# flatironinstitute/bayes-kit

Measured on NVIDIA B200. Metric: hmc_chain_steps_per_s, higher is better.
Workload: dtype f32

## Files before the change

bayes-kit_b200/csrc/dense_tc.cu:

```cuda
#include <cuda.h>
#include <cuda_bf16.h>
#include <stdio.h>
#include <stdlib.h>

#include <mutex>

#include "dense_tc.h"
#include "sep_common.cuh"

namespace bk {

namespace tc {

constexpr int BM = 128;
constexpr int BN = 256;
constexpr int BK = 64;
constexpr int UK = 16;
constexpr int CWID = 16;
constexpr int EDEPTH_MAX = 4;
constexpr int ECHUNK_BYTES = 2 * CWID * 32 * 4;
template <int MODE, bool PAIR = false> struct Cfg {
    static constexpr int KS = MODE == TC_MODE_STEP ? 32 : 64;
#ifndef BK_STEP_STAGES
#define BK_STEP_STAGES 8
// ... 505 lines not shown
                                const float qn = qj + fmaf(em2, gj, qj - pj);
                                __stcs(qw + j * BM, qn);
                                const __nv_bfloat16 hi = __float2bfloat16_rn(qn);
                                hw[j * BK] = hi;
                                lw[j * BK] = __float2bfloat16_rn(qn - __bfloat162float(hi));
                            }
                        }
                    } else if (!no_mem) {
#pragma unroll
                        for (int j = 0; j < CWID; ++j) {
                            float pj, qj;
                            asm volatile("ld.shared.f32 %0, [%1];" : "=f"(pj) : "r"(src + j * 128));
                            asm volatile("ld.shared.f32 %0, [%1];" : "=f"(qj) : "r"(src + CWID * 128 + j * 128));
                            if (d_ok && cbase + ch * CWID + j < a.C) {
                                const float gj = cv - __uint_as_float(v[j]);
                                const float qn = qj + fmaf(em2, gj, qj - pj);
                                __stcs(qw + j * BM, qn);
                                const __nv_bfloat16 hi = __float2bfloat16_rn(qn);
                                hw[j * BK] = hi;
                                if (lw) lw[j * BK] = __float2bfloat16_rn(qn - __bfloat162float(hi));
                            }
                        }
                    }
                    qw += CWID * BM;
                    hw += CWID * BK;
                    if (lw) lw += CWID * BK;
                    src += ECHUNK_BYTES;
                    if (++slot == EDEPTH) { slot = 0; src -= EDEPTH * ECHUNK_BYTES; }
                    __syncwarp();
                };
                static_assert(NC % 2 == 0, "two register sets ping-pong");
                uint32_t va[CWID], vb[CWID];
                const bool no_tmem = (a.debug & 16) != 0;
                if (!no_tmem) tmem_ld16_async(t0, va);
#pragma unroll 1
                for (int ch = 0; ch < NC; ch += 2) {
                    issue();
                    cp_async_wait<EDEPTH - 1>();
                    __syncwarp();
                    tmem_wait_ld16(va);
                    if (!no_tmem) tmem_ld16_async(t0 + (ch + 1) * CWID, vb);
                    process(va, ch);
                    issue();
                    cp_async_wait<EDEPTH - 1>();
                    __syncwarp();
                    tmem_wait_ld16(vb);
                    if (ch + 2 < NC && !no_tmem) tmem_ld16_async(t0 + (ch + 2) * CWID, va);
                    process(vb, ch + 1);
                }
                if (!d_ok && !no_mem) {
                    hw -= NC * CWID * BK;
                    if (lw) lw -= NC * CWID * BK;
                    for (int j = 0; j < NCH * 32; ++j)
                        if (cbase + j < a.C) {
                            hw[(int64_t)j * BK] = __float2bfloat16_rn(0.f);
                            if (lw) lw[(int64_t)j * BK] = __float2bfloat16_rn(0.f);
                        }
                }
                tc_fence_before();
                if constexpr (PAIR) {
                    if (step < n_steps - 1) fence_proxy_async_global();
                    __syncwarp();
                    if (lane == 0) {
                        mbar_arrive_cluster(mapa_rank(tempty(acc), 0));
                        if (step < n_steps - 1) mbar_arrive(twritten(sig_k));
                    }
                    ++sig_k;
                } else {
                    mbar_arrive(tempty(acc));
                }
                if (++acc == 2) { acc = 0; acc_phase ^= 1u; }
            }
            cp_async_wait<0>();
        }
    }
    tc_fence_before();
    __syncthreads();
    if constexpr (PAIR) cluster_sync_all();
    if (warp == 1) {
        tc_fence_after();
        if constexpr (PAIR)
            asm volatile("tcgen05.dealloc.cta_group::2.sync.aligned.b32 %0, %1;" ::"r"(tmem_base), "r"(TMEM_COLS)
                         : "memory");
        else
            asm volatile("tcgen05.dealloc.cta_group::1.sync.aligned.b32 %0, %1;" ::"r"(tmem_base), "r"(TMEM_COLS)
                         : "memory");
    }
}

__global__ void k_split_matrix(const float* __restrict__ P, int D, int Dp, __nv_bfloat16* __restrict__ hi,
                               __nv_bfloat16* __restrict__ lo) {
    int64_t i = (int64_t)blockIdx.x * blockDim.x + threadIdx.x;
    if (i >= (int64_t)Dp * Dp) return;
    int r = (int)(i / Dp), c = (int)(i % Dp);
    float v = (r < D && c < D) ? P[(int64_t)r * D + c] : 0.0f;
    __nv_bfloat16 h = __float2bfloat16_rn(v);
    const int64_t o = box_index(r, c, Dp / BK, BM);
    hi[o] = h;
    lo[o] = __float2bfloat16_rn(v - __bfloat162float(h));
}

__global__ void k_pmu(const float* __restrict__ P, const float* __restrict__ mu, int D, float* __restrict__ out) {
    int r = (int)(((int64_t)blockIdx.x * blockDim.x + threadIdx.x) >> 5), lane = threadIdx.x & 31;
    if (r >= D) return;
    double s = 0;
    for (int k = lane; k < D; k += 32) s += (double)P[(int64_t)r * D + k] * (double)mu[k];
    s = warp_sum(s);
    if (lane == 0) out[r] = (float)s;
}

__global__ void k_split_rows(const float* __restrict__ x, int64_t C, int D, int Dp,
                             __nv_bfloat16* __restrict__ hi, __nv_bfloat16* __restrict__ lo) {
    int64_t i = (int64_t)blockIdx.x * blockDim.x + threadIdx.x;
    if (i >= C * Dp) return;
    int64_t c = i / Dp;
    int d = (int)(i % Dp);
    float v = d < D ? x[c * D + d] : 0.f;
    __nv_bfloat16 h = __float2bfloat16_rn(v);
    const int64_t o = box_index(c, d, Dp / BK, BN);
    hi[o] = h;
    if (lo) lo[o] = __float2bfloat16_rn(v - __bfloat162float(h));
}

struct HmcTcArgs {
    float *theta, *lp, *grad;
    float *q, *qm, *gq, *h0;
    __nv_bfloat16 *q_hi, *q_lo;
    const float *metric, *mu;
    int64_t C;
    int D, Dp, L, m_tiles;
    float eps, half_eps, inv_eps;
    bk_rng rng;
    float *draws, *logp;
    int32_t* accept;
    int out_lp;
    const uint32_t* err;
    const float *qs, *gs;
    int old_blocked;
    __nv_bfloat16 *nq_hi, *nq_lo;
};

template <bool VEC>
__device__ __forceinline__ void ld4(const float* p, int e, int D, float (&v)[4]) {
    if (VEC) {
        const float4 t = *reinterpret_cast<const float4*>(p + e);
        v[0] = t.x; v[1] = t.y; v[2] = t.z; v[3] = t.w;
    } else {
#pragma unroll
        for (int i = 0; i < 4; ++i) v[i] = (e + i < D) ? p[e + i] : 0.f;
    }
}
template <bool VEC>
__device__ __forceinline__ void st4(float* p, int e, int D, const float (&v)[4]) {
    if (VEC) {
        *reinterpret_cast<float4*>(p + e) = make_float4(v[0], v[1], v[2], v[3]);
    } else {
#pragma unroll
        for (int i = 0; i < 4; ++i)
            if (e + i < D) p[e + i] = v[i];
    }
}
template <bool VEC>
__device__ __forceinline__ void st4_bf16(__nv_bfloat16* p, int e, int D, const __nv_bfloat16 (&v)[4]) {
    if (VEC) {
        uint2 u;
        u.x = (uint32_t)__bfloat16_as_ushort(v[0]) | ((uint32_t)__bfloat16_as_ushort(v[1]) << 16);
        u.y = (uint32_t)__bfloat16_as_ushort(v[2]) | ((uint32_t)__bfloat16_as_ushort(v[3]) << 16);
        *reinterpret_cast<uint2*>(p + e) = u;
    } else {
#pragma unroll
        for (int i = 0; i < 4; ++i)
            if (e + i < D) p[e + i] = v[i];
    }
}

template <bool VEC>
__global__ void __launch_bounds__(256) k_hmc_begin_tc(HmcTcArgs p, int64_t t, int write_lo) {
    const int64_t c = ((int64_t)blockIdx.x * blockDim.x + threadIdx.x) >> 5;
    const int lane = threadIdx.x & 31;
    if (c >= p.C) return;
    const int D = p.D;
    const int64_t off = c * (int64_t)D;
    float kin = 0.f;
#pragma unroll 2
    for (int b = lane; 4 * b < D; b += 32) {
        const int e = 4 * b;
        float z[4], g[4], th[4], m[4] = {1.f, 1.f, 1.f, 1.f};
        ld4<VEC>(p.grad + off, e, D, g);
        ld4<VEC>(p.theta + off, e, D, th);
        if (p.metric) ld4<VEC>(p.metric, e, D, m);
        if (p.rng.mode == BK_RNG_INJECTED)
            ld4<VEC>(reinterpret_cast<const float*>(p.rng.normals) + (t * p.C + c) * (int64_t)D, e, D, z);
        else
            philox_normal4<float>(p.rng.seed, (uint32_t)b, (uint32_t)(p.rng.chain_offset + (uint64_t)c),
                                  (uint32_t)(p.rng.draw_offset + (uint64_t)t), z);
        float r[4], q[4];
        __nv_bfloat16 hi[4], lo[4];
#pragma unroll
        for (int i = 0; i < 4; ++i) {
            if (!VEC && e + i >= D) z[i] = 0.f;
            const float mg = m[i] * g[i];
            kin = fmaf(z[i], m[i] * z[i], kin);
            r[i] = z[i] - p.half_eps * mg;
            r[i] = r[i] + p.eps * mg;
            q[i] = th[i] + p.eps * r[i];
            hi[i] = __float2bfloat16_rn(q[i]);
            lo[i] = __float2bfloat16_rn(q[i] - __bfloat162float(hi[i]));
        }
        const int64_t bo = blk_index(c, e, p.m_tiles);
        st4<true>(p.qm + bo, 0, 4, th);
        st4<true>(p.q + bo, 0, 4, q);
        const int64_t xo = box_index(c, e, p.Dp / BK, BN);
        st4_bf16<true>(p.q_hi + xo, 0, 4, hi);
        if (write_lo) st4_bf16<true>(p.q_lo + xo, 0, 4, lo);
    }
    for (int b = (D + 3) / 4 + lane; 4 * b < p.Dp; b += 32) {
        const __nv_bfloat16 zero4[4] = {__float2bfloat16_rn(0.f), __float2bfloat16_rn(0.f), __float2bfloat16_rn(0.f),
                                        __float2bfloat16_rn(0.f)};
        const int64_t xo = box_index(c, 4 * b, p.Dp / BK, BN);
        st4_bf16<true>(p.q_hi + xo, 0, 4, zero4);
        if (write_lo) st4_bf16<true>(p.q_lo + xo, 0, 4, zero4);
    }
    kin = warp_sum(kin);
    if (lane == 0) p.h0[c] = p.lp[c] - 0.5f * kin;
}

template <bool VEC>
__global__ void __launch_bounds__(256) k_hmc_end_tc(HmcTcArgs p, int64_t t) {
    const int64_t c = ((int64_t)blockIdx.x * blockDim.x + threadIdx.x) >> 5;
    const int lane = threadIdx.x & 31;
    if (c >= p.C) return;
    const int D = p.D;
    const int64_t off = c * (int64_t)D;
    float kin = 0.f, dot = 0.f;
#pragma unroll 2
    for (int b = lane; 4 * b < D; b += 32) {
        const int e = 4 * b;
        float g[4], qm[4], q[4], m[4] = {1.f, 1.f, 1.f, 1.f}, mu[4] = {0.f, 0.f, 0.f, 0.f};
        const int64_t bo = blk_index(c, e, p.m_tiles);
        ld4<true>(p.gq + bo, 0, 4, g);
        ld4<true>(p.qm + bo, 0, 4, qm);
        ld4<true>(p.q + bo, 0, 4, q);
        if (p.metric) ld4<VEC>(p.metric, e, D, m);
        if (p.mu) ld4<VEC>(p.mu, e, D, mu);
#pragma unroll
        for (int i = 0; i < 4; ++i) {
            if (e + i >= D) break;
            const float rf = fmaf(q[i] - qm[i], p.inv_eps, p.half_eps * (m[i] * g[i]));
            kin = fmaf(rf, m[i] * rf, kin);
            dot = fmaf(q[i] - mu[i], g[i], dot);
        }
    }
    kin = warp_sum(kin);
    dot = warp_sum(dot);
    const bool lost = p.err && *p.err != 0u;
    const float lpq = lost ? __int_as_float(0x7fc00000) : 0.5f * dot;
    const float h1 = lpq - 0.5f * kin, h0 = lost ? lpq : p.h0[c];
    float u;
    if (p.rng.mode == BK_RNG_INJECTED)
        u = reinterpret_cast<const float*>(p.rng.uniforms)[(t * p.C + c) * p.rng.n_uniform];
    else
        u = philox_accept_uniform<float>(p.rng.seed, (uint32_t)(p.rng.chain_offset + (uint64_t)c),
                                         (uint32_t)(p.rng.draw_offset + (uint64_t)t), D);
    const bool acc = log_u(u) < h1 - h0;
    float* dr = p.draws ? p.draws + (t * p.C + c) * (int64_t)D : nullptr;
#pragma unroll 2
    for (int b = lane; 4 * b < D; b += 32) {
        const int e = 4 * b;
        float v[4];
        if (acc) {
            float g[4];
            const int64_t bo = blk_index(c, e, p.m_tiles);
            ld4<true>(p.q + bo, 0, 4, v);
            ld4<true>(p.gq + bo, 0, 4, g);
            st4<VEC>(p.theta + off, e, D, v);
            st4<VEC>(p.grad + off, e, D, g);
        } else if (p.old_blocked) {
            float g[4];
            const int64_t bo = blk_index(c, e, p.m_tiles);
            ld4<true>(p.qs + bo, 0, 4, v);
            ld4<true>(p.gs + bo, 0, 4, g);
            st4<VEC>(p.theta + off, e, D, v);
            st4<VEC>(p.grad + off, e, D, g);
        } else if (dr) {
            ld4<VEC>(p.theta + off, e, D, v);
        }
        if (dr) st4<VEC>(dr, e, D, v);
    }
    if (lane == 0) {
        const float lp_old = p.lp[c];
        if (acc) p.lp[c] = lpq;
        if (p.logp) p.logp[t * p.C + c] = p.out_lp ? (acc ? lpq : lp_old) : (acc ? h1 : h0);
        if (p.accept) p.accept[t * p.C + c] = acc ? 1 : 0;
    }
}

template <bool VEC>
__global__ void __launch_bounds__(256, 4) k_hmc_turn_tc(HmcTcArgs p, int64_t t, int write_lo) {
    const int64_t c = ((int64_t)blockIdx.x * blockDim.x + threadIdx.x) >> 5;
    const int lane = threadIdx.x & 31;
    if (c >= p.C) return;
    const int D = p.D;
    const int64_t off = c * (int64_t)D;
    float kin = 0.f, dot = 0.f;
#pragma unroll 2
    for (int b = lane; 4 * b < D; b += 32) {
        const int e = 4 * b;
        float g[4], qm[4], q[4], m[4] = {1.f, 1.f, 1.f, 1.f}, mu[4] = {0.f, 0.f, 0.f, 0.f};
        const int64_t bo = blk_index(c, e, p.m_tiles);
        ld4<true>(p.gq + bo, 0, 4, g);
        ld4<true>(p.qm + bo, 0, 4, qm);
        ld4<true>(p.q + bo, 0, 4, q);
        if (p.metric) ld4<VEC>(p.metric, e, D, m);
        if (p.mu) ld4<VEC>(p.mu, e, D, mu);
#pragma unroll
        for (int i = 0; i < 4; ++i) {
            if (e + i >= D) break;
            const float rf = fmaf(q[i] - qm[i], p.inv_eps, p.half_eps * (m[i] * g[i]));
            kin = fmaf(rf, m[i] * rf, kin);
            dot = fmaf(q[i] - mu[i], g[i], dot);
        }
    }
    kin = warp_sum(kin);
    dot = warp_sum(dot);
    const bool lost = p.err && *p.err != 0u;
    const float lpq = lost ? __int_as_float(0x7fc00000) : 0.5f * dot;
    const float h1 = lpq - 0.5f * kin, h0 = lost ? lpq : p.h0[c];
    float u;
    if (p.rng.mode == BK_RNG_INJECTED)
        u = reinterpret_cast<const float*>(p.rng.uniforms)[(t * p.C + c) * p.rng.n_uniform];
    else
        u = philox_accept_uniform<float>(p.rng.seed, (uint32_t)(p.rng.chain_offset + (uint64_t)c),
                                         (uint32_t)(p.rng.draw_offset + (uint64_t)t), D);
    const bool acc = log_u(u) < h1 - h0;
    float* dr = p.draws ? p.draws + (t * p.C + c) * (int64_t)D : nullptr;
    float kin0 = 0.f;
#pragma unroll 2
    for (int b = lane; 4 * b < D; b += 32) {
        const int e = 4 * b;
        const int64_t bo = blk_index(c, e, p.m_tiles);
        float v[4], g[4], z[4], m[4] = {1.f, 1.f, 1.f, 1.f};
        if (acc) {
            ld4<true>(p.q + bo, 0, 4, v);
            ld4<true>(p.gq + bo, 0, 4, g);
        } else {
            if (p.old_blocked) {
                ld4<true>(p.qs + bo, 0, 4, v);
                ld4<true>(p.gs + bo, 0, 4, g);
            } else {
                ld4<VEC>(p.theta + off, e, D, v);
                ld4<VEC>(p.grad + off, e, D, g);
            }
            st4<true>(p.q + bo, 0, 4, v);
            st4<true>(p.gq + bo, 0, 4, g);
        }
        if (dr) st4<VEC>(dr, e, D, v);
        if (p.metric) ld4<VEC>(p.metric, e, D, m);
        if (p.rng.mode == BK_RNG_INJECTED)
            ld4<VEC>(reinterpret_cast<const float*>(p.rng.normals) + ((t + 1) * p.C + c) * (int64_t)D, e, D, z);
        else
            philox_normal4<float>(p.rng.seed, (uint32_t)b, (uint32_t)(p.rng.chain_offset + (uint64_t)c),
                                  (uint32_t)(p.rng.draw_offset + (uint64_t)(t + 1)), z);
        float q1[4];
        __nv_bfloat16 hi[4], lo[4];
#pragma unroll
        for (int i = 0; i < 4; ++i) {
            if (e + i >= D) { z[i] = 0.f; v[i] = 0.f; g[i] = 0.f; }
            const float mg = m[i] * g[i];
            kin0 = fmaf(z[i], m[i] * z[i], kin0);
            float r = z[i] - p.half_eps * mg;
            r = r + p.eps * mg;
            q1[i] = v[i] + p.eps * r;
            hi[i] = __float2bfloat16_rn(q1[i]);
            lo[i] = __float2bfloat16_rn(q1[i] - __bfloat162float(hi[i]));
        }
        st4<true>(p.qm + bo, 0, 4, q1);
        const int64_t xo = box_index(c, e, p.Dp / BK, BN);
        st4_bf16<true>(p.nq_hi + xo, 0, 4, hi);
        if (write_lo) st4_bf16<true>(p.nq_lo + xo, 0, 4, lo);
    }
    for (int b = (D + 3) / 4 + lane; 4 * b < p.Dp; b += 32) {
        const __nv_bfloat16 zero4[4] = {__float2bfloat16_rn(0.f), __float2bfloat16_rn(0.f), __float2bfloat16_rn(0.f),
                                        __float2bfloat16_rn(0.f)};
        const int64_t xo = box_index(c, 4 * b, p.Dp / BK, BN);
        st4_bf16<true>(p.nq_hi + xo, 0, 4, zero4);
        if (write_lo) st4_bf16<true>(p.nq_lo + xo, 0, 4, zero4);
    }
    kin0 = warp_sum(kin0);
    if (lane == 0) {
        const float lp_old = p.lp[c];
        const float lp_new = acc ? lpq : lp_old;
        if (acc) p.lp[c] = lpq;
        p.h0[c] = lp_new - 0.5f * kin0;
        if (p.logp) p.logp[t * p.C + c] = p.out_lp ? lp_new : (acc ? h1 : h0);
        if (p.accept) p.accept[t * p.C + c] = acc ? 1 : 0;
    }
}

typedef CUresult (*EncodeFn)(CUtensorMap*, CUtensorMapDataType, cuuint32_t, void*, const cuuint64_t*,
                             const cuuint64_t*, const cuuint32_t*, const cuuint32_t*, CUtensorMapInterleave,
                             CUtensorMapSwizzle, CUtensorMapL2promotion, CUtensorMapFloatOOBfill);

static EncodeFn get_encode() {
    static EncodeFn fn = nullptr;
    if (!fn) {
        void* p = nullptr;
        cudaDriverEntryPointQueryResult q;
        if (cudaGetDriverEntryPoint("cuTensorMapEncodeTiled", &p, cudaEnableDefault, &q) == cudaSuccess &&
            q == cudaDriverEntryPointSuccess)
            fn = (EncodeFn)p;
    }
    return fn;
}

static int make_map(CUtensorMap* m, const void* ptr, int64_t rows, int Dp, int box_rows, int box_k, int blk_rows = 0) {
    EncodeFn enc = get_encode();
    if (!enc) { set_error("cuTensorMapEncodeTiled is unavailable (driver too old?)"); return BK_E_CUDA; }
    if (!blk_rows) blk_rows = box_rows;
    const int64_t row_tiles = (rows + blk_rows - 1) / blk_rows;
    cuuint64_t dims[2] = {(cuuint64_t)BK, (cuuint64_t)(row_tiles * (Dp / BK) * blk_rows)};
    cuuint64_t strides[1] = {(cuuint64_t)BK * 2};
    cuuint32_t box[2] = {(cuuint32_t)box_k, (cuuint32_t)box_rows};
    cuuint32_t el[2] = {1, 1};
    CUresult r = enc(m, CU_TENSOR_MAP_DATA_TYPE_BFLOAT16, 2, const_cast<void*>(ptr), dims, strides, box, el,
                     CU_TENSOR_MAP_INTERLEAVE_NONE,
                     box_k == 64 ? CU_TENSOR_MAP_SWIZZLE_128B : CU_TENSOR_MAP_SWIZZLE_64B,
                     CU_TENSOR_MAP_L2_PROMOTION_L2_256B, CU_TENSOR_MAP_FLOAT_OOB_FILL_NONE);
    if (r != CUDA_SUCCESS) { set_error("cuTensorMapEncodeTiled failed (%d)", (int)r); return BK_E_CUDA; }
    return BK_OK;
}

constexpr int MAX_FUSED_STEPS = 64;

static int max_fused_steps(int m_tiles, int debug) {
    static int fuse_env = -1, pair_env = -1;
    static int clusters_dev[64], sms_dev[64];
    static bool dev_init = false;
    static std::mutex dev_mu;
    std::lock_guard<std::mutex> dev_lock(dev_mu);
    if (!dev_init) { for (int i = 0; i < 64; ++i) { clusters_dev[i] = -1; sms_dev[i] = 0; } dev_init = true; }
    int cur_dev = 0;
    if (cudaGetDevice(&cur_dev) != cudaSuccess || cur_dev < 0 || cur_dev >= 64) return 1;
    int& clusters = clusters_dev[cur_dev];
    int& sms = sms_dev[cur_dev];
    if (fuse_env < 0) { const char* e = getenv("BK_TC_FUSE"); fuse_env = (e && e[0] == '0') ? 0 : 1; }
    if (pair_env < 0) { const char* e = getenv("BK_TC_PAIR"); pair_env = (e && e[0] == '0') ? 0 : 1; }
    if (!fuse_env || !pair_env || m_tiles % 2 != 0 || (debug & 4)) return 1;
    if (clusters < 0) {
        int dev = 0;
        if (cudaGetDevice(&dev) != cudaSuccess ||
            cudaDeviceGetAttribute(&sms, cudaDevAttrMultiProcessorCount, dev) != cudaSuccess) return 1;
        cudaFuncSetAttribute(k_dense_tc<TC_MODE_STEP, true>, cudaFuncAttributeMaxDynamicSharedMemorySize,
                             Cfg<TC_MODE_STEP, true>::SMEM_BYTES);
        cudaLaunchConfig_t cfg;
        memset(&cfg, 0, sizeof(cfg));
        cfg.gridDim = dim3(2u * (unsigned)(sms / 2));
        cfg.blockDim = dim3(THREADS);
        cfg.dynamicSmemBytes = Cfg<TC_MODE_STEP, true>::SMEM_BYTES;
        cudaLaunchAttribute at[1];
        at[0].id = cudaLaunchAttributeClusterDimension;
        at[0].val.clusterDim.x = 2; at[0].val.clusterDim.y = 1; at[0].val.clusterDim.z = 1;
        cfg.attrs = at;
        cfg.numAttrs = 1;
        int n = 0;
        if (cudaOccupancyMaxActiveClusters(&n, k_dense_tc<TC_MODE_STEP, true>, &cfg) != cudaSuccess) { cudaGetLastError(); n = 0; }
        clusters = n;
    }
    return clusters >= sms / 2 ? MAX_FUSED_STEPS : 1;
}

static int launch_tc(const Model& m, const StepArgs& a, const __nv_bfloat16* b_hi, const __nv_bfloat16* b_lo,
                     cudaStream_t st) {
    static bool attr_dev[64] = {false};
    static int sms_by_dev[64] = {0};
    int launch_dev = 0;
    BK_CUDA(cudaGetDevice(&launch_dev));
    if (launch_dev < 0 || launch_dev >= 64) { set_error("device index %d out of range", launch_dev); return BK_E_CUDA; }
    bool& attr = attr_dev[launch_dev];
    if (!attr) {
        BK_CUDA(cudaFuncSetAttribute(k_dense_tc<TC_MODE_STEP, false>, cudaFuncAttributeMaxDynamicSharedMemorySize,
                                     Cfg<TC_MODE_STEP, false>::SMEM_BYTES));
        BK_CUDA(cudaFuncSetAttribute(k_dense_tc<TC_MODE_GRAD, false>, cudaFuncAttributeMaxDynamicSharedMemorySize,
                                     Cfg<TC_MODE_GRAD, false>::SMEM_BYTES));
        BK_CUDA(cudaFuncSetAttribute(k_dense_tc<TC_MODE_STEP, true>, cudaFuncAttributeMaxDynamicSharedMemorySize,
                                     Cfg<TC_MODE_STEP, true>::SMEM_BYTES));
        BK_CUDA(cudaFuncSetAttribute(k_dense_tc<TC_MODE_GRAD, true>, cudaFuncAttributeMaxDynamicSharedMemorySize,
                                     Cfg<TC_MODE_GRAD, true>::SMEM_BYTES));
        attr = true;
    }
    static int pair_env = -1;
    if (pair_env < 0) { const char* e = getenv("BK_TC_PAIR"); pair_env = (e && e[0] == '0') ? 0 : 1; }
    const bool pair = pair_env && a.m_tiles % 2 == 0 && !(a.debug & 4);
    int& sms = sms_by_dev[launch_dev];
    if (!sms) BK_CUDA(cudaDeviceGetAttribute(&sms, cudaDevAttrMultiProcessorCount, launch_dev));
    CUtensorMap mA0, mA1, mB0, mB1;
    int rc;
    const int bk = a.mode == TC_MODE_STEP ? Cfg<TC_MODE_STEP>::KS : Cfg<TC_MODE_GRAD>::KS;
    if ((rc = make_map(&mA0, m.P_hi, m.Dp, (int)m.Dp, BM, bk))) return rc;
    if ((rc = make_map(&mA1, m.P_lo, m.Dp, (int)m.Dp, BM, bk))) return rc;
    const int brows = pair ? BN / 2 : BN;
    if ((rc = make_map(&mB0, b_hi, a.C, (int)m.Dp, brows, bk, BN))) return rc;
    const __nv_bfloat16* b1 = a.n_steps > 1 ? a.q_hi_next : (b_lo ? b_lo : b_hi);
    if ((rc = make_map(&mB1, b1, a.C, (int)m.Dp, brows, bk, BN))) return rc;
    if (a.n_steps > 1 && !(pair && a.mode == TC_MODE_STEP)) { set_error("fused steps need the pair STEP kernel"); return BK_E_INVALID; }
    const int tag = a.mode == TC_MODE_STEP ? BK_PROF_STEP : BK_PROF_GRAD;
    if (pair) {
        const int64_t units = a.n_tiles * (a.m_tiles / 2);
        const int64_t max_pairs = sms / 2;
        const unsigned grid = 2u * (unsigned)(units < max_pairs ? units : max_pairs);
        cudaLaunchConfig_t cfg;
        memset(&cfg, 0, sizeof(cfg));
        cfg.gridDim = dim3(grid);
        cfg.blockDim = dim3(THREADS);
        cfg.stream = st;
        cudaLaunchAttribute at[1];
        at[0].id = cudaLaunchAttributeClusterDimension;
        at[0].val.clusterDim.x = 2; at[0].val.clusterDim.y = 1; at[0].val.clusterDim.z = 1;
        cfg.attrs = at;
        cfg.numAttrs = 1;
        static std::mutex fused_mu;
        static cudaEvent_t fused_ev[64] = {nullptr};
        std::unique_lock<std::mutex> fused_lock(fused_mu, std::defer_lock);
        int fused_dev = -1;
        if (a.n_steps > 1) {
            fused_lock.lock();
            BK_CUDA(cudaGetDevice(&fused_dev));
            if (fused_dev < 0 || fused_dev >= 64) { set_error("device index %d out of range", fused_dev); return BK_E_CUDA; }
            if (!fused_ev[fused_dev]) BK_CUDA(cudaEventCreateWithFlags(&fused_ev[fused_dev], cudaEventDisableTiming));
            else BK_CUDA(cudaStreamWaitEvent(st, fused_ev[fused_dev], 0));
            BK_CUDA(cudaMemsetAsync(a.sync, 0, (size_t)(a.n_steps - 1) * a.n_tiles * sizeof(uint32_t), st));
        }
        prof_begin(tag, st);
        cudaError_t e;
        if (a.mode == TC_MODE_STEP) {
            cfg.dynamicSmemBytes = Cfg<TC_MODE_STEP, true>::SMEM_BYTES;
            e = cudaLaunchKernelEx(&cfg, k_dense_tc<TC_MODE_STEP, true>, mA0, mA1, mB0, mB1, a);
            if (fused_dev >= 0 && e == cudaSuccess) e = cudaEventRecord(fused_ev[fused_dev], st);

        } else {
            cfg.dynamicSmemBytes = Cfg<TC_MODE_GRAD, true>::SMEM_BYTES;
            e = cudaLaunchKernelEx(&cfg, k_dense_tc<TC_MODE_GRAD, true>, mA0, mA1, mB0, mB1, a);
        }
        prof_end(tag, st);
        if (e != cudaSuccess) { set_error("pair launch failed: %s", cudaGetErrorString(e)); return BK_E_CUDA; }
        count_launch();
        return BK_OK;
    }
    const int64_t tiles = a.n_tiles * a.m_tiles;
    const unsigned grid = (unsigned)(tiles < sms ? tiles : sms);
    prof_begin(tag, st);
    if (a.mode == TC_MODE_STEP)
        k_dense_tc<TC_MODE_STEP, false><<<grid, THREADS, Cfg<TC_MODE_STEP, false>::SMEM_BYTES, st>>>(mA0, mA1, mB0, mB1, a);
    else
        k_dense_tc<TC_MODE_GRAD, false><<<grid, THREADS, Cfg<TC_MODE_GRAD, false>::SMEM_BYTES, st>>>(mA0, mA1, mB0, mB1, a);
    prof_end(tag, st);
    BK_LAUNCH_CHECK();
    return BK_OK;
}

}

bool dense_tc_enabled(const Model& m) {
    const char* e = getenv("BK_DISABLE_TC");
    if (e && e[0] == '1') return false;
    return m.d.kind == BK_MODEL_DENSE_PREC_GAUSS && m.d.dtype == BK_F32 && m.P_hi != nullptr;
}

size_t dense_tc_model_ws_bytes(const bk_model_desc& d) {
    if (d.kind != BK_MODEL_DENSE_PREC_GAUSS || d.dtype != BK_F32) return 0;
    const size_t Dp = align_up((size_t)d.dims, 128);
    return 2 * align_up(Dp * Dp * 2, 256) + align_up((size_t)d.dims * 4, 256) + 1024;
}

int dense_tc_prepare(Model& m, void* ws, size_t ws_bytes, cudaStream_t st) {
    if (m.d.kind != BK_MODEL_DENSE_PREC_GAUSS || m.d.dtype != BK_F32) return BK_OK;
    const int D = (int)m.d.dims;
    m.Dp = (int64_t)align_up((size_t)D, 128);
    Arena ar(ws, ws_bytes);
    m.P_hi = ar.take<__nv_bfloat16>((size_t)m.Dp * m.Dp);
    m.P_lo = ar.take<__nv_bfloat16>((size_t)m.Dp * m.Dp);
    m.Pmu = m.d.mu ? (void*)ar.take<float>(D) : nullptr;
    if (!ar.ok()) {
        m.P_hi = m.P_lo = nullptr;
        m.Pmu = nullptr;
        set_error("bk_model_create: workspace too small for the tensor-core operands (%zu < %zu)", ws_bytes,
                  ar.off);
        return BK_E_WORKSPACE;
    }
    const int64_t n = m.Dp * m.Dp;
    tc::k_split_matrix<<<(unsigned)((n + 255) / 256), 256, 0, st>>>((const float*)m.d.P, D, (int)m.Dp, m.P_hi,
                                                                     m.P_lo);
    BK_LAUNCH_CHECK();
    if (m.Pmu) {
        tc::k_pmu<<<(unsigned)(((int64_t)D * 32 + 255) / 256), 256, 0, st>>>((const float*)m.d.P,
                                                                             (const float*)m.d.mu, D,
                                                                             (float*)m.Pmu);
        BK_LAUNCH_CHECK();
    }
    return BK_OK;
}

size_t dense_tc_hmc_ws_bytes(const Model& m, int64_t C) {
    const size_t n = (size_t)align_up((size_t)C, tc::BN) * m.Dp;
    const size_t nb = n;
    const size_t n_tiles = align_up((size_t)C, tc::BN) / tc::BN;
    return 5 * align_up(n * 4, 256) + align_up((size_t)C * 4, 256) + 3 * align_up(nb * 2, 256) +
           align_up(tc::MAX_FUSED_STEPS * n_tiles * 4 + 256, 256) + model_eval_ws_bytes(m, C) + 2048;
}

int dense_tc_grad(const Model& m, const float* theta, int64_t C, float* grad, void* ws, size_t ws_bytes,
                  cudaStream_t st) {
    Arena ar(ws, ws_bytes);
    const size_t nb = (size_t)align_up((size_t)C, tc::BN) * m.Dp;
    __nv_bfloat16* hi = ar.take<__nv_bfloat16>(nb);
    __nv_bfloat16* lo = ar.take<__nv_bfloat16>(nb);
    if (!ar.ok()) { set_error("dense_tc_grad: workspace too small"); return BK_E_WORKSPACE; }
    const int D = (int)m.d.dims;
    tc::k_split_rows<<<(unsigned)((C * m.Dp + 255) / 256), 256, 0, st>>>(theta, C, D, (int)m.Dp, hi, lo);
    BK_LAUNCH_CHECK();
    tc::StepArgs a;
    memset(&a, 0, sizeof(a));
    a.mode = TC_MODE_GRAD; a.n_pass = 3; a.C = C; a.D = D; a.Dp = (int)m.Dp;
    a.m_tiles = (int)(m.Dp / tc::BM); a.n_tiles = (C + tc::BN - 1) / tc::BN; a.kblocks = (int)(m.Dp / tc::BK);
    a.cvec = (const float*)m.Pmu; a.g_out = grad;
    return tc::launch_tc(m, a, hi, lo, st);
}

int dense_tc_hmc(const Model& m, float* theta, float* lp, float* grad, int32_t* cache_valid, int64_t C,
                 double eps, int L, const float* metric, int64_t n_draws, const bk_rng* rng,
                 const bk_draw_out& out, void* ws, size_t ws_bytes, cudaStream_t st, bool report_lp) {
    const int D = (int)m.d.dims;
    const size_t n = (size_t)align_up((size_t)C, tc::BN) * m.Dp;
    const size_t nb = n;
    Arena ar(ws, ws_bytes);
    float* Q[3] = {ar.take<float>(n), ar.take<float>(n), ar.take<float>(n)};
    float* G[2] = {ar.take<float>(n), ar.take<float>(n)};
    float* h0 = ar.take<float>(C);
    __nv_bfloat16* qhi[2] = {ar.take<__nv_bfloat16>(nb), ar.take<__nv_bfloat16>(nb)};
    __nv_bfloat16* qlo = ar.take<__nv_bfloat16>(nb);
    uint32_t* sync = ar.take<uint32_t>(tc::MAX_FUSED_STEPS * (align_up((size_t)C, tc::BN) / tc::BN) + 64);
    uint32_t* err_word = sync + tc::MAX_FUSED_STEPS * (align_up((size_t)C, tc::BN) / tc::BN);
    const size_t ebytes = model_eval_ws_bytes(m, C);
    void* ews = ar.take<char>(ebytes);
    if (!ar.ok()) {
        set_error("bk_hmc_diag_sample: workspace too small (need %zu bytes, got %zu)", ar.off, ws_bytes);
        return BK_E_WORKSPACE;
    }
    int rc;
    if (!cache_valid || !*cache_valid) {
        rc = model_eval(m, theta, C, lp, grad, ews, ebytes, st);
        if (rc) return rc;
        if (cache_valid) *cache_valid = 1;
    }
    tc::HmcTcArgs h;
    memset(&h, 0, sizeof(h));
    h.theta = theta; h.lp = lp; h.grad = grad; h.h0 = h0;
    h.metric = metric; h.mu = (const float*)m.d.mu; h.C = C; h.D = D; h.Dp = (int)m.Dp; h.L = L;
    h.m_tiles = (int)(m.Dp / tc::BM);
    h.eps = (float)eps; h.half_eps = (float)(0.5 * eps); h.inv_eps = (float)(1.0 / eps); h.rng = *rng;
    h.draws = (float*)out.draws; h.logp = (float*)out.logp; h.accept = out.accept;
    h.out_lp = report_lp ? 1 : 0;
    h.err = err_word;
    BK_CUDA(cudaMemsetAsync(err_word, 0, sizeof(uint32_t), st));
    tc::StepArgs a;
    memset(&a, 0, sizeof(a));
    a.err = err_word;
    a.C = C; a.D = D; a.Dp = (int)m.Dp;
    a.m_tiles = (int)(m.Dp / tc::BM); a.n_tiles = (C + tc::BN - 1) / tc::BN; a.kblocks = (int)(m.Dp / tc::BK);
    a.eps = (float)eps; a.metric = metric; a.cvec = (const float*)m.Pmu;
    a.g_blocked = 1;
    { const char* e = getenv("BK_TC_DEBUG"); a.debug = e ? atoi(e) : 0; }
    static int turn_env = -1;
    if (turn_env < 0) { const char* e = getenv("BK_TC_TURN"); turn_env = (e && e[0] == '0') ? 0 : 1; }
    const unsigned wblocks = (unsigned)((C * 32 + 255) / 256);
    auto al16 = [](const void* p) { return (reinterpret_cast<uintptr_t>(p) & 15) == 0; };
    const bool vec = D % 4 == 0 && al16(theta) && al16(grad) && al16(metric) && al16(m.d.mu) &&
                     al16(out.draws) && (rng->mode != BK_RNG_INJECTED || al16(rng->normals));
    int x = 0, y = 1, z = 2, ga = 0, gb = 1;
    bool state_blocked = false, begun = false;
    for (int64_t t = 0; t < n_draws; ++t) {
        if (!begun) {
            h.q_hi = qhi[0]; h.q_lo = qlo;
            h.qm = Q[x]; h.q = Q[y];
            if (vec) tc::k_hmc_begin_tc<true><<<wblocks, 256, 0, st>>>(h, t, L == 1 ? 1 : 0);
            else tc::k_hmc_begin_tc<false><<<wblocks, 256, 0, st>>>(h, t, L == 1 ? 1 : 0);
            BK_LAUNCH_CHECK();
        }
        int cur = 0, iprev = x, icur = y;
        bool first = true;
        const int max_fuse = tc::max_fused_steps(a.m_tiles, a.debug);
        for (int s = 1; s < L;) {
// ... 52 lines not shown
```

Before: 21.19 million.

## Speculatively start next HMC trajectory in first pass, redo only on rejection

The turn kernel now computes the next trajectory's first leapfrog position, draw and bf16 split during the energy-reduction pass, assuming the proposal is accepted. A second pass over the state runs only when the proposal is rejected, or when qm aliases qs. Next-row loads are software-prefetched one iteration ahead. This avoids re-reading q, gq and metric and recomputing the RNG on accepted steps, but rejected steps now do the work twice.

```diff
diff --git a/bayes-kit_b200/csrc/dense_tc.cu b/bayes-kit_b200/csrc/dense_tc.cu
--- a/bayes-kit_b200/csrc/dense_tc.cu
+++ b/bayes-kit_b200/csrc/dense_tc.cu
@@ -831,15 +831,51 @@
     if (c >= p.C) return;
     const int D = p.D;
     const int64_t off = c * (int64_t)D;
-    float kin = 0.f, dot = 0.f;
-#pragma unroll 2
+    float* dr = p.draws ? p.draws + (t * p.C + c) * (int64_t)D : nullptr;
+    const bool q1_late = p.old_blocked && p.qm == p.qs;
+    auto start = [&](int b, int64_t bo, float (&v)[4], float (&g)[4], const float (&m)[4], bool store_q1,
+                     float* kin0) {
+        const int e = 4 * b;
+        float z[4];
+        if (p.rng.mode == BK_RNG_INJECTED)
+            ld4<VEC>(reinterpret_cast<const float*>(p.rng.normals) + ((t + 1) * p.C + c) * (int64_t)D, e, D, z);
+        else
+            philox_normal4<float>(p.rng.seed, (uint32_t)b, (uint32_t)(p.rng.chain_offset + (uint64_t)c),
+                                  (uint32_t)(p.rng.draw_offset + (uint64_t)(t + 1)), z);
+        float q1[4];
+        __nv_bfloat16 hi[4], lo[4];
+#pragma unroll
+        for (int i = 0; i < 4; ++i) {
+            if (e + i >= D) { z[i] = 0.f; v[i] = 0.f; g[i] = 0.f; }
+            const float mg = m[i] * g[i];
+            if (kin0) *kin0 = fmaf(z[i], m[i] * z[i], *kin0);
+            float r = z[i] - p.half_eps * mg;
+            r = r + p.eps * mg;
+            q1[i] = v[i] + p.eps * r;
+            hi[i] = __float2bfloat16_rn(q1[i]);
+            lo[i] = __float2bfloat16_rn(q1[i] - __bfloat162float(hi[i]));
+        }
+        if (store_q1) st4<true>(p.qm + bo, 0, 4, q1);
+        const int64_t xo = box_index(c, e, p.Dp / BK, BN);
+        st4_bf16<true>(p.nq_hi + xo, 0, 4, hi);
+        if (write_lo) st4_bf16<true>(p.nq_lo + xo, 0, 4, lo);
+    };
+    float kin = 0.f, dot = 0.f, kin0 = 0.f;
+    float g[4], qm[4], q[4];
+    auto load_rows = [&](int b, float (&g_)[4], float (&qm_)[4], float (&q_)[4]) {
+        const int64_t bo = blk_index(c, 4 * b, p.m_tiles);
+        ld4<true>(p.gq + bo, 0, 4, g_);
+        ld4<true>(p.qm + bo, 0, 4, qm_);
+        ld4<true>(p.q + bo, 0, 4, q_);
+    };
+    if (4 * lane < D) load_rows(lane, g, qm, q);
+#pragma unroll 1
     for (int b = lane; 4 * b < D; b += 32) {
         const int e = 4 * b;
-        float g[4], qm[4], q[4], m[4] = {1.f, 1.f, 1.f, 1.f}, mu[4] = {0.f, 0.f, 0.f, 0.f};
+        float gn[4], qmn[4], qn[4], m[4] = {1.f, 1.f, 1.f, 1.f}, mu[4] = {0.f, 0.f, 0.f, 0.f};
         const int64_t bo = blk_index(c, e, p.m_tiles);
-        ld4<true>(p.gq + bo, 0, 4, g);
-        ld4<true>(p.qm + bo, 0, 4, qm);
-        ld4<true>(p.q + bo, 0, 4, q);
+        const bool more = 4 * (b + 32) < D;
+        if (more) load_rows(b + 32, gn, qmn, qn);
         if (p.metric) ld4<VEC>(p.metric, e, D, m);
         if (p.mu) ld4<VEC>(p.mu, e, D, mu);
 #pragma unroll
@@ -849,9 +885,23 @@
             kin = fmaf(rf, m[i] * rf, kin);
             dot = fmaf(q[i] - mu[i], g[i], dot);
         }
+        if (dr) st4<VEC>(dr, e, D, q);
+        start(b, bo, q, g, m, !q1_late, &kin0);
+        if (more) {
+#pragma unroll
+            for (int i = 0; i < 4; ++i) { g[i] = gn[i]; qm[i] = qmn[i]; q[i] = qn[i]; }
+        }
+    }
+    for (int b = (D + 3) / 4 + lane; 4 * b < p.Dp; b += 32) {
+        const __nv_bfloat16 zero4[4] = {__float2bfloat16_rn(0.f), __float2bfloat16_rn(0.f), __float2bfloat16_rn(0.f),
+                                        __float2bfloat16_rn(0.f)};
+        const int64_t xo = box_index(c, 4 * b, p.Dp / BK, BN);
+        st4_bf16<true>(p.nq_hi + xo, 0, 4, zero4);
+        if (write_lo) st4_bf16<true>(p.nq_lo + xo, 0, 4, zero4);
     }
     kin = warp_sum(kin);
     dot = warp_sum(dot);
+    kin0 = warp_sum(kin0);
     const bool lost = p.err && *p.err != 0u;
     const float lpq = lost ? __int_as_float(0x7fc00000) : 0.5f * dot;
     const float h1 = lpq - 0.5f * kin, h0 = lost ? lpq : p.h0[c];
@@ -862,60 +912,30 @@
         u = philox_accept_uniform<float>(p.rng.seed, (uint32_t)(p.rng.chain_offset + (uint64_t)c),
                                          (uint32_t)(p.rng.draw_offset + (uint64_t)t), D);
     const bool acc = log_u(u) < h1 - h0;
-    float* dr = p.draws ? p.draws + (t * p.C + c) * (int64_t)D : nullptr;
-    float kin0 = 0.f;
-#pragma unroll 2
-    for (int b = lane; 4 * b < D; b += 32) {
-        const int e = 4 * b;
-        const int64_t bo = blk_index(c, e, p.m_tiles);
-        float v[4], g[4], z[4], m[4] = {1.f, 1.f, 1.f, 1.f};
-        if (acc) {
-            ld4<true>(p.q + bo, 0, 4, v);
-            ld4<true>(p.gq + bo, 0, 4, g);
-        } else {
-            if (p.old_blocked) {
-                ld4<true>(p.qs + bo, 0, 4, v);
-                ld4<true>(p.gs + bo, 0, 4, g);
+    if (!acc || q1_late) {
+        for (int b = lane; 4 * b < D; b += 32) {
+            const int e = 4 * b;
+            const int64_t bo = blk_index(c, e, p.m_tiles);
+            float v[4], g[4], m[4] = {1.f, 1.f, 1.f, 1.f};
+            if (acc) {
+                ld4<true>(p.q + bo, 0, 4, v);
+                ld4<true>(p.gq + bo, 0, 4, g);
             } else {
-                ld4<VEC>(p.theta + off, e, D, v);
-                ld4<VEC>(p.grad + off, e, D, g);
+                if (p.old_blocked) {
+                    ld4<true>(p.qs + bo, 0, 4, v);
+                    ld4<true>(p.gs + bo, 0, 4, g);
+                } else {
+                    ld4<VEC>(p.theta + off, e, D, v);
+                    ld4<VEC>(p.grad + off, e, D, g);
+                }
+                st4<true>(p.q + bo, 0, 4, v);
+                st4<true>(p.gq + bo, 0, 4, g);
+                if (dr) st4<VEC>(dr, e, D, v);
             }
-            st4<true>(p.q + bo, 0, 4, v);
-            st4<true>(p.gq + bo, 0, 4, g);
-        }
-        if (dr) st4<VEC>(dr, e, D, v);
-        if (p.metric) ld4<VEC>(p.metric, e, D, m);
-        if (p.rng.mode == BK_RNG_INJECTED)
-            ld4<VEC>(reinterpret_cast<const float*>(p.rng.normals) + ((t + 1) * p.C + c) * (int64_t)D, e, D, z);
-        else
-            philox_normal4<float>(p.rng.seed, (uint32_t)b, (uint32_t)(p.rng.chain_offset + (uint64_t)c),
-                                  (uint32_t)(p.rng.draw_offset + (uint64_t)(t + 1)), z);
-        float q1[4];
-        __nv_bfloat16 hi[4], lo[4];
-#pragma unroll
-        for (int i = 0; i < 4; ++i) {
-            if (e + i >= D) { z[i] = 0.f; v[i] = 0.f; g[i] = 0.f; }
-            const float mg = m[i] * g[i];
-            kin0 = fmaf(z[i], m[i] * z[i], kin0);
-            float r = z[i] - p.half_eps * mg;
-            r = r + p.eps * mg;
-            q1[i] = v[i] + p.eps * r;
-            hi[i] = __float2bfloat16_rn(q1[i]);
-            lo[i] = __float2bfloat16_rn(q1[i] - __bfloat162float(hi[i]));
-        }
-        st4<true>(p.qm + bo, 0, 4, q1);
-        const int64_t xo = box_index(c, e, p.Dp / BK, BN);
-        st4_bf16<true>(p.nq_hi + xo, 0, 4, hi);
-        if (write_lo) st4_bf16<true>(p.nq_lo + xo, 0, 4, lo);
-    }
-    for (int b = (D + 3) / 4 + lane; 4 * b < p.Dp; b += 32) {
-        const __nv_bfloat16 zero4[4] = {__float2bfloat16_rn(0.f), __float2bfloat16_rn(0.f), __float2bfloat16_rn(0.f),
-                                        __float2bfloat16_rn(0.f)};
-        const int64_t xo = box_index(c, 4 * b, p.Dp / BK, BN);
-        st4_bf16<true>(p.nq_hi + xo, 0, 4, zero4);
-        if (write_lo) st4_bf16<true>(p.nq_lo + xo, 0, 4, zero4);
-    }
-    kin0 = warp_sum(kin0);
+            if (p.metric) ld4<VEC>(p.metric, e, D, m);
+            start(b, bo, v, g, m, true, nullptr);
+        }
+    }
     if (lane == 0) {
         const float lp_old = p.lp[c];
         const float lp_new = acc ? lpq : lp_old;
```

After: 21.35 million (median of 6 runs). Within noise of the previous version (+0.7%).
